# richarddurbin/hash10x

Measured on AMD Instinct MI355X. Metric: read-pairs/s through --readFQB + --hashDepthRange + --cluster (mosh construction + per-barcode clustering), higher is better.
Workload: dtype u64; 1 GPU; yeast-like-2.5M; read_pairs=2500000, barcodes=10000, B=24, k=21, w=31, clusterThreshold=5, parallelism=single GPU

## Files before the change

### hash10x_amd/csrc/stage_c.hip

```cpp
#include "common.hpp"
#include <chrono>
#include "prim.hpp"
#include <type_traits>
#include <rocprim/block/block_radix_sort.hpp>

namespace h10x {


constexpr int CL_THREADS_SMALL = 1024;
constexpr int CL_THREADS_HUGE = 1024;
constexpr u16 NONE16 = 0xFFFF;
constexpr u32 NOHANDLE = 0xFFFFFFFFu;
constexpr int ROWS_IN_FLIGHT = 4;
constexpr int RCHUNK = 4;

__global__ void within_kernel(const u32 *__restrict__ depth, u32 hashNumber, int lo, int hi, u8 *__restrict__ within) {
  const u32 i = blockIdx.x * blockDim.x + threadIdx.x;
  if (i >= hashNumber) return;
  const int n = (int)depth[i];
  if (n >= lo && n < hi) within[i] = 1;
}
__global__ void within_depth_kernel(const u32 *__restrict__ depth, const u8 *__restrict__ within, u32 hashNumber, u32 *__restrict__ out,
                                    const u64 *__restrict__ rowStart, u32 rowShift, u64 *__restrict__ rowInfo ) {
  const u32 i = blockIdx.x * blockDim.x + threadIdx.x;
// ... 182 lines not shown
  const u16 *goodPos; const u32 *nGood;
  const u64 *goodRow;
  const u32 *rows;
  const u32 *list; u32 nList; u32 *workCounter;
  u32 *started;
  const u32 *front; u32 nFront;
  u32 nBlocks; int threshold;
  SegMap segs;
  u32 rowShift;
  u32 nBlocksFirst;
  u32 firstCap;
  u32 hashMinSlots;
  u32 hashBits;
  u16 *handles; size_t handleStride; u32 hStride;
  const u32 *entries;
  u32 *overflow, *overflowCount;
  unsigned char *scratch; size_t scratchStride;
  u32 maxGood;
  u32 ldsBudget;
  u64 *res;
  u64 *stats;
  u64 *phase;
  u32 narrowFirst;
  u32 tpClassT;
};

#define RES_PACK(best, q, tot) ((u64)(best) | ((u64)(q) << 16) | ((u64)(tot) << 40))
constexpr u32 RES_COUNT_MAX = (1u << 24) - 1;
struct Work {
  u16 *first;
  u32 *bm; u16 *pre;
  u16 *root;
  u32 *hist;
  u32 histWords;
};
__host__ __device__ inline size_t pad16(size_t b) { return (b + 15) & ~(size_t)15; }
__host__ __device__ inline size_t workBytes(u32 nFirst, u32 n, u32 nWaves, u32 bmWords) {
  size_t b = pad16((size_t)nFirst * 2) + pad16((size_t)bmWords * 4) + pad16((size_t)bmWords * 2);
  b += pad16((size_t)n * 2);
  b += (size_t)nWaves * (((size_t)n + 3) / 4) * 4;
  return b + 16;
}
constexpr u32 MIN_HIST_WAVES = 5;
constexpr u32 RANKED_FIRST_PER_RANK = 6;
__host__ __device__ inline u32 rankedFirstEstimate(u32 nBarcodes, u32 n) { const u64 e = (u64)RANKED_FIRST_PER_RANK * n; return e < nBarcodes ? (u32)e : nBarcodes; }
__host__ __device__ inline u32 rankedFirstEstimateE(u32 nBarcodes, u32 n, u32 entries, u32 div = 7) { const u32 a = rankedFirstEstimate(nBarcodes, n), b = entries / div; const u32 m = a > b ? a : b; return m < nBarcodes ? m : nBarcodes; }
__host__ __device__ inline u32 histWaves(u32 nFirst, u32 n, u32 maxWaves, u32 bmWords, size_t budget) {
  const size_t fixed = workBytes(nFirst, n, 0, bmWords), per = (((size_t)n + 3) / 4) * 4;
  if (fixed + MIN_HIST_WAVES * per > budget) return 0;
  const size_t wv = (budget - fixed) / (per ? per : 1);
  return wv < maxWaves ? (u32)wv : maxWaves;
}
__device__ inline Work carve(unsigned char *base, u32 nFirst, u32 n, u32 bmWords = 0) {
  Work w; size_t o = 0;
  w.first = (u16 *)(base + o); o += pad16((size_t)nFirst * 2);
  w.bm = (u32 *)(base + o); o += pad16((size_t)bmWords * 4);
  w.pre = (u16 *)(base + o); o += pad16((size_t)bmWords * 2);
  w.root = (u16 *)(base + o); o += pad16((size_t)n * 2);
  w.hist = (u32 *)(base + o); w.histWords = (n + 3) / 4;
  return w;
}
__host__ __device__ inline size_t mergeBytes(u32 nRep) {
  return (((size_t)nRep + 15) & ~(size_t)15) + 256 * 8 * 4 + 256 * 4 + 512 * 4 + 16;
}

template <bool IN_LDS, typename T> __device__ __forceinline__ T ld_shared(const T *p) {
  if (IN_LDS) return *p;
  return __hip_atomic_load(p, __ATOMIC_RELAXED, __HIP_MEMORY_SCOPE_AGENT);
}

template <bool IN_LDS>
__device__ __forceinline__ void min_u16(u16 *arr, u32 idx, u32 val) {
  u32 *w = (u32 *)arr + (idx >> 1); const int sh = (idx & 1) * 16;
  u32 old = ld_shared<IN_LDS>(w);
  for (;;) {
    if (((old >> sh) & 0xFFFFu) <= val) return;
    const u32 nw = (old & ~(0xFFFFu << sh)) | (val << sh);
    const u32 prev = atomicCAS(w, old, nw);
    if (prev == old) return;
    old = prev;
  }
}

template <bool FIRST_LDS> struct FirstDense {
  static constexpr bool MASK_TAIL = false;
  static constexpr bool SELF = true;
  u32 none;
  u16 *first; u32 wide;
  __device__ __forceinline__ u32 update(u32 cj, u32 i) const {
    if (FIRST_LDS && wide) atomicMin(&((u32 *)first)[cj], i); else min_u16<FIRST_LDS>(first, cj, i);
    return cj;
  }
  __device__ __forceinline__ u32 peek(u32 h) const {
    if (FIRST_LDS) return *(const u16 *)((const unsigned char *)first + (u32)(h << (1 + wide)));
    return ld_shared<FIRST_LDS>(&first[h]);
  }
  __device__ __forceinline__ u32 lookup(u32 cj) const { return peek(cj); }
  __device__ __forceinline__ u32 entry(const void *row, u32 j, u32 code) const { const u32 cj = ((const u32 *)row)[j]; return cj != code ? lookup(cj) : (u32)NONE16; }
};
struct FirstRanked {
  static constexpr bool SELF = false;
  static constexpr bool MASK_TAIL = false;
  u16 *first; const u32 *bm; const u16 *pre; u32 wide;
  u32 none;
  __device__ __forceinline__ u32 at(u32 cj) const { const u32 w = cj >> 5; return pre[w] + (u32)__popc(bm[w] & ((1u << (cj & 31)) - 1u)); }
  __device__ __forceinline__ u32 update(u32 cj, u32 i) const { const u32 h = at(cj); if (wide) atomicMin(&((u32 *)first)[h], i); else min_u16<true>(first, h, i); return h; }
  __device__ __forceinline__ u32 peek(u32 h) const { return *(const u16 *)((const unsigned char *)first + (u32)(h << (1 + wide))); }
  __device__ __forceinline__ u32 lookup(u32 cj) const { return peek(at(cj)); }
  __device__ __forceinline__ u32 entry(const void *row, u32 j, u32 code) const { const u32 cj = ((const u32 *)row)[j]; return cj != code ? lookup(cj) : (u32)NONE16; }
};
constexpr u32 TR_QUEUE = 16384;
constexpr u32 TR_MIN_SLOTS = 1024;
constexpr u32 TR_MAX_SLOTS = 65532;
struct SlotTable {
  u32 *tab; u32 NB , xsh , tsh; u32 *ovf; u32 hbase ;
  u32 base3;
  typedef __attribute__((address_space(3))) u32 lds_u32;
  typedef u32 u32x4 __attribute__((ext_vector_type(4)));
  typedef __attribute__((address_space(3))) u32x4 lds_u32x4;
  static constexpr u32 SCRAMBLE = 0x9E3779u;
  static constexpr u32 MAXD = 63;
  static constexpr u32 NOTFOUND = 0xFFFFFFFFu;
  __device__ __forceinline__ void shape(u32 *t, u32 slots, u32 hashBits, u32 *o, u32 hb) {
    tab = t; NB = slots / 4; xsh = 32 - hashBits; ovf = o; hbase = hb; base3 = 0;
    const u32 lg = 31 - (u32)__clz((int)NB), x = 32 - hashBits + lg; tsh = x < 31 ? x : 31;
  }
  __device__ __forceinline__ void inLds() { base3 = (u32)(size_t)(lds_u32 *)tab; }
  __device__ __forceinline__ u32 search(u32 cj, u32 i, bool insert, bool &ins) const {
    const u32 x = __umul24(cj, SCRAMBLE) << xsh;
    u32 b = __umulhi(x, NB);
    const u32 tag = (x * NB) >> tsh;
    const u32 step = 2 * (tag & 7u) + 1;
    ins = false;
    for (u32 key = tag; key < (MAXD << 10); key += 1u << 10) {
      const u32 mine = (i << 16) | key;
      const uint4 e4 = *(const uint4 *)&tab[4 * b];
      const u32 e[4] = {e4.x, e4.y, e4.z, e4.w};
      u32 hit = 4, eh = 0;
#pragma unroll
      for (int w = 3; w >= 0; --w) { const bool m = (e[w] & 0xFFFFu) == key; hit = m ? (u32)w : hit; eh = m ? e[w] : eh; }
      if (hit < 4) { if (eh > (mine | 0xFFFFu)) atomicMin(&tab[4 * b + hit], mine); return hbase + 4 * b + hit; }
#pragma unroll
      for (int w = 0; w < 4; ++w)
        if (e[w] == 0xFFFFFFFFu) {
          if (!insert) return NOTFOUND;
          const u32 old = atomicCAS(&tab[4 * b + w], 0xFFFFFFFFu, mine);
          if (old == 0xFFFFFFFFu) { ins = true; return hbase + 4 * b + w; }
          if ((old & 0xFFFFu) == key) { if (old > (mine | 0xFFFFu)) atomicMin(&tab[4 * b + w], mine); return hbase + 4 * b + w; }
        }
      b += step; if (b >= NB) b -= NB;
    }
    if (insert) *ovf = 1;
    return NOTFOUND;
  }
  __device__ __forceinline__ bool probeHome(u32 cj, u32 i, bool valid , bool insert, u32 &slot, bool &ins) const {
    const u32 x = __umul24(cj, SCRAMBLE) << xsh;
    const u32 b4 = __umulhi(x, NB) << 2;
    const u32 key = (x * NB) >> tsh;
    const u32 mine = (i << 16) | key;
    const u32 aBucket = base3 + (b4 << 2);
    const u32x4 e4 = *(const lds_u32x4 *)(uintptr_t)aBucket;
    const bool m0 = (e4.x & 0xFFFFu) == key, m1 = (e4.y & 0xFFFFu) == key, m2 = (e4.z & 0xFFFFu) == key, m3 = (e4.w & 0xFFFFu) == key;
    const bool z0 = e4.x == 0xFFFFFFFFu, z1 = e4.y == 0xFFFFFFFFu, z2 = e4.z == 0xFFFFFFFFu, z3 = e4.w == 0xFFFFFFFFu;
    const bool hit = m0 | m1 | m2 | m3;
    const u32 wh = m0 ? 0u : (m1 ? 1u : (m2 ? 2u : 3u)), wz = z0 ? 0u : (z1 ? 1u : (z2 ? 2u : 3u));
    const u32 word = hit ? wh : wz;
    slot = b4 | word;
    lds_u32 *const pSlot = (lds_u32 *)(uintptr_t)(aBucket + (word << 2));
    const bool claim = valid && !hit && insert && (z0 | z1 | z2 | z3);
    u32 seen = 0xFFFFFFFEu;
    if (claim) { u32 expect = 0xFFFFFFFFu; __hip_atomic_compare_exchange_strong(pSlot, &expect, mine, __ATOMIC_RELAXED, __ATOMIC_RELAXED, __HIP_MEMORY_SCOPE_WORKGROUP); seen = expect; }
    ins = seen == 0xFFFFFFFFu;
    const bool same = (seen & 0xFFFFu) == key;
    if ((valid && hit) || same) (void)__hip_atomic_fetch_min(pSlot, mine, __ATOMIC_RELAXED, __HIP_MEMORY_SCOPE_WORKGROUP);
    return !valid || hit || ins || same;
  }
};
struct FirstSlots {
  static constexpr bool SELF = false;
  static constexpr bool MASK_TAIL = false;
  const unsigned char *base; u32 sh;
  u32 none;
  __device__ __forceinline__ u32 peek(u32 h) const { return *(const u16 *)(base + (u32)(h << sh)); }
  __device__ __forceinline__ u32 lookup(u32 h) const { return peek(h); }
// ... 89 lines not shown
      }
    }
  if (RCHUNK > 1) {
#pragma unroll
    for (int r = 0; r < RCHUNK; ++r)
      if ((u32)(r * WAVE) < d && ok[r]) {
        if (IN_LDS) hist[f[r] >> 2] = 0;
        else atomicAnd(&hist[f[r] >> 2], 0u);
      }
  }
  if (!(RCHUNK > 2) || __builtin_amdgcn_ballot_w64(key >= (thr << 16))) {
    key = wave_max_u32(key);
    bcnt = key >> 16;
    best = key ? 0xFFFFu - (key & 0xFFFFu) : NONE16;
    if (bcnt >= thr) {
      rb = ld_shared<IN_LDS>(&root[best]);
      if (rb != NONE16) {
#pragma unroll
        for (int r = 0; r < RCHUNK; ++r) if ((u32)(r * WAVE) < d) q += (u32)__popcll(__ballot(f[r] == rb));
      }
    }
  }
}
template <typename FT>
__device__ __forceinline__ u32 row_count_value(const void *__restrict__ row, u32 d, u32 code, u32 i, const FT &ft, u32 v, u32 &tot) {
  const int lane = threadIdx.x & (WAVE - 1);
  u32 q = 0; tot = 0;
  for (u32 b0 = 0; b0 < d; b0 += WAVE) {
    u32 f = NONE16;
    if (b0 + lane < d) f = ft.entry(row, b0 + lane, code);
    q += (u32)__popcll(__ballot(f == v && v != NONE16)); tot += (u32)__popcll(__ballot(f < i));
  }
  return q;
}
template <typename FT>
__device__ __forceinline__ void row_mode_long(const void *__restrict__ row, u32 d, u32 code, u32 i, const FT &ft, u32 &best, u32 &bcnt, u32 &tot) {
  const int lane = threadIdx.x & (WAVE - 1);
  best = NONE16; bcnt = 0; tot = 0;
  for (u32 a0 = 0; a0 < d; a0 += WAVE) {
    u32 fa = NONE16; bool va = false;
    if (a0 + lane < d) { fa = ft.entry(row, a0 + lane, code); va = fa < i; }
    u64 rem = __ballot(va); tot += (u32)__popcll(rem);
    while (rem) {
      const int src = __ffsll((long long)rem) - 1;
      const u32 v = (u32)__builtin_amdgcn_readlane((int)fa, src);
      rem &= ~__ballot(fa == v);
      u32 cnt = 0; bool seenBefore = false;
      for (u32 b0 = 0; b0 < d; b0 += WAVE) {
        u32 fb = NONE16;
        if (b0 + lane < d) fb = ft.entry(row, b0 + lane, code);
        const u32 m = (u32)__popcll(__ballot(fb == v));
        if (b0 < a0 && m) { seenBefore = true; break; }
        cnt += m;
      }
      if (!seenBefore && (cnt > bcnt || (cnt == bcnt && v < best))) { bcnt = cnt; best = v; }
    }
  }
}
#define STAMP(k) do { if (a.phase && threadIdx.x == 0) { const u64 t__ = wall_clock64(); atomicAdd((u64 *)&a.phase[k], t__ - (u64)acc.s[4]); acc.s[4] = t__; } } while (0)

#define SYNC() do { __syncthreads(); if (!IN_LDS) __builtin_amdgcn_fence(__ATOMIC_ACQUIRE, "agent"); } while (0)
#define SYNC_LDS() do { if (IN_LDS) { __builtin_amdgcn_fence(__ATOMIC_RELEASE, "workgroup"); asm volatile("s_waitcnt lgkmcnt(0)\n\ts_barrier" ::: "memory"); __builtin_amdgcn_fence(__ATOMIC_ACQUIRE, "workgroup"); } else SYNC(); } while (0)

struct Desc { u32 x , y ; };
__device__ __forceinline__ Desc descLane(u32 v, int t) { Desc d; d.x = (u32)__builtin_amdgcn_readlane((int)v, t); d.y = (u32)__builtin_amdgcn_readlane((int)v, 32 + t); return d; }
__device__ __forceinline__ u32 descLoad(const u64 *gr, u32 i0, u32 nLists, u32 n) {
  const u32 lane = threadIdx.x & (WAVE - 1), t = lane & 31, i = i0 + t;
  return (t < nLists && i >= 1 && i < n) ? ((const u32 *)gr)[2 * (size_t)i + (lane >> 5)] : 0u;
}

__device__ __forceinline__ u32 descLoadU(const u64 *gr, u32 i0, u32 n) {
  const u32 lane = threadIdx.x & (WAVE - 1), i = i0 + (lane & 31);
  return ((const u32 *)gr)[2 * (size_t)(i < n ? i : n - 1) + (lane >> 5)];
}
__device__ __forceinline__ u32 descFix(u32 v, u32 i0, u32 nLists, u32 n) {
  const u32 lane = threadIdx.x & (WAVE - 1), t = lane & 31, i = i0 + t;
  return (lane < 32 || (t < nLists && i >= 1 && i < n)) ? v : 0u;
}

template <int CL_THREADS> __device__ __forceinline__ void fill16(void *p, size_t bytes, u32 v) {
  const uint4 v4 = make_uint4(v, v, v, v);
  for (u32 i = threadIdx.x; i < (u32)(bytes / 16); i += CL_THREADS) ((uint4 *)p)[i] = v4;
}
struct WorkAcc { u32 depth; unsigned long long *s; };
template <bool IN_LDS, int FIRST_MODE , int CL_THREADS, int KLASS>
__device__ __forceinline__ void cluster_one_block(const ClusterArgs &a, u32 code, unsigned char *region, u16 *firstGlobal, u32 *sh , WorkAcc &acc) {
  constexpr int CL_WAVES = CL_THREADS / WAVE;
  constexpr int RIF = (KLASS == 0 && CL_THREADS == 1024 && FIRST_MODE == 1) ? 2 : ROWS_IN_FLIGHT;
  const int tid = threadIdx.x, lane = tid & (WAVE - 1), wave = tid / WAVE;
  code = (u32)__builtin_amdgcn_readfirstlane((int)code);
  const u32 n = (u32)__builtin_amdgcn_readfirstlane((int)a.nGood[code]);
  if (n == 0) return;
  const u64 o = a.blockOff[code];
  constexpr bool FIRST_LDS = IN_LDS && FIRST_MODE != 2;
  constexpr bool RANKED = IN_LDS && FIRST_MODE == 1;
  const u32 bmWords = RANKED ? (a.nBlocksFirst + 31) / 32 : 0;
  u32 nW;
  if constexpr (RANKED) nW = 0;
  else nW = IN_LDS ? histWaves(FIRST_LDS ? a.nBlocksFirst : 0, n, CL_WAVES, bmWords, a.ldsBudget) : (u32)CL_WAVES;
  if (!RANKED && !nW) return;
  bool wideFirst = false;
  if (FIRST_LDS && !RANKED && a.narrowFirst != 1) {
    const u32 nW4 = histWaves(2 * a.nBlocksFirst, n, CL_WAVES, bmWords, a.ldsBudget);
    wideFirst = nW4 >= nW || (a.narrowFirst >= 2 && nW4 >= a.narrowFirst);
    if (wideFirst) nW = nW4;
  }
  Work w = carve(region, RANKED ? 0 : (FIRST_LDS || !IN_LDS ? (wideFirst ? 2 * a.nBlocksFirst : a.nBlocksFirst) : 0), n, bmWords);
  if (IN_LDS && FIRST_MODE == 2) w.first = firstGlobal;
  typename std::conditional<RANKED, FirstRanked, FirstDense<FIRST_LDS>>::type ft{};
  if constexpr (RANKED) { ft.first = w.first; ft.bm = w.bm; ft.pre = w.pre; ft.wide = 0; }
  else { ft.first = w.first; ft.wide = wideFirst ? 1u : 0u; }
  const u32 lcode = code; code = a.segs.globalOf(lcode);
  if constexpr (!RANKED) ft.none = code;
  const u32 rsh = a.rowShift;
#define ROWP(rs) (a.rows + ((size_t)(rs) << rsh))
  const u64 *const gr = a.goodRow + o;
  u64 *const res = a.res + o;
  const u32 thr = (u32)a.threshold;

  if (a.phase && threadIdx.x == 0) acc.s[4] = wall_clock64();
  if (FIRST_LDS && !RANKED) {
    if (wideFirst) fill16<CL_THREADS>(w.first, pad16((size_t)a.nBlocksFirst * 4), (u32)NONE16);
    else fill16<CL_THREADS>(w.first, pad16((size_t)a.nBlocksFirst * 2), 0xFFFFFFFFu);
  }
  if (RANKED) fill16<CL_THREADS>(w.bm, pad16((size_t)bmWords * 4), 0u);
  if (!RANKED) fill16<CL_THREADS>(w.hist, pad16((size_t)nW * w.histWords * 4), 0u);
  fill16<CL_THREADS>(w.root, pad16((size_t)n * 2), 0xFFFFFFFFu);
  if (tid == 0) { w.root[0] = 0; res[0] = RES_PACK(NONE16, 0, 0); }
  SYNC();
  if constexpr (RANKED) {
    typedef __attribute__((address_space(3))) u32 lds_u32;
    lds_u32 *const bm3 = (lds_u32 *)w.bm;
    auto mark = [&](u32 cj) { if (cj != code) __hip_atomic_fetch_or(&bm3[cj >> 5], 1u << (cj & 31), __ATOMIC_RELAXED, __HIP_MEMORY_SCOPE_WORKGROUP); };
    constexpr int BIF = 8;
    const u32 uw = (u32)__builtin_amdgcn_readfirstlane(wave);
    u32 dvN = descLoad(gr, 1 + uw * BIF, BIF, n);
    for (u32 i0 = 1 + uw * BIF; i0 < n; i0 += CL_WAVES * BIF) {
      u32 c0[BIF], c1[BIF], d4[BIF], r4[BIF];
      const u32 dv = dvN;
      dvN = descLoad(gr, i0 + CL_WAVES * BIF, BIF, n);
#pragma unroll
      for (int t = 0; t < BIF; ++t) {
        const Desc g2 = descLane(dv, t);
        d4[t] = g2.y; r4[t] = g2.x;
        const u32 *row = ROWP(r4[t]);
        c0[t] = (u32)lane < d4[t] ? row[lane] : code; c1[t] = (u32)(WAVE + lane) < d4[t] ? row[WAVE + lane] : code;
      }
#pragma unroll
      for (int t = 0; t < BIF; ++t) {
        mark(c0[t]);
        if (d4[t] > WAVE) {
          mark(c1[t]);
          if (d4[t] > 2 * WAVE) { const u32 *row = ROWP(r4[t]); for (u32 j = 2 * WAVE + lane; j < d4[t]; j += WAVE) mark(row[j]); }
        }
      }
    }
    SYNC();
    const u32 ipt = (bmWords + CL_THREADS - 1) / CL_THREADS, s0 = tid * ipt < bmWords ? tid * ipt : bmWords, s1 = s0 + ipt < bmWords ? s0 + ipt : bmWords;
    u32 mine = 0;
    for (u32 q = s0; q < s1; ++q) mine += (u32)__popc(w.bm[q]);
    u32 inc = mine;
#pragma unroll
    for (int dd = 1; dd < WAVE; dd <<= 1) { const u32 o2 = (u32)__shfl_up((int)inc, dd); if (lane >= dd) inc += o2; }
    if (lane == WAVE - 1) sh[4 + wave] = inc;
    SYNC();
    u32 run = inc - mine, total = 0;
    for (int q = 0; q < CL_WAVES; ++q) { if (q < wave) run += sh[4 + q]; total += sh[4 + q]; }
    for (u32 q = s0; q < s1; ++q) { w.pre[q] = (u16)run; run += (u32)__popc(w.bm[q]); }
    {
      const size_t fixed = workBytes(0, n, 0, bmWords), per = (size_t)w.histWords * 4, need = pad16((size_t)total * 2) + 32;
      const bool fits = total <= 65535u && fixed + need + MIN_HIST_WAVES * per <= a.ldsBudget && !(a.firstCap && total > a.firstCap);
      if (!fits) {
        if (tid == 0) a.overflow[atomicAdd(a.overflowCount, 1u)] = lcode;
        SYNC();
        return;
      }
      const size_t wv = (a.ldsBudget - fixed - need) / (per ? per : 1);
      nW = wv < (size_t)CL_WAVES ? (u32)wv : (u32)CL_WAVES;
      const size_t need4 = pad16((size_t)total * 4) + 32;
      ft.wide = (a.narrowFirst != 1 && fixed + need4 + (size_t)nW * per <= a.ldsBudget) ? 1u : 0u;
      w.first = (u16 *)((unsigned char *)w.hist + pad16((size_t)nW * per));
      ft.first = w.first;
    }
    for (u32 i = tid; i < nW * w.histWords; i += CL_THREADS) w.hist[i] = 0;
    ft.none = total;
    if (ft.wide) for (u32 q = tid; q <= total; q += CL_THREADS) ((u32 *)w.first)[q] = NONE16;
    else for (u32 q = tid; q < (total + 2) / 2; q += CL_THREADS) ((u32 *)w.first)[q] = 0xFFFFFFFFu;
    SYNC();
  }
  STAMP(0);

#define H10X_LOAD_D(I0, DV) { DV = descLoad(gr, (I0), RIF, n); }
#define H10X_LOAD_A(CJ, DV)                                                                                   \
  { _Pragma("unroll") for (int t = 0; t < RIF; ++t) { const Desc g2 = descLane(DV, t); CJ[t] = (u32)lane < g2.y ? ROWP(g2.x)[lane] : code; } }
#define H10X_LOAD_B(CJ2, DV)                                                                                  \
  { _Pragma("unroll") for (int t = 0; t < RIF; ++t) { const Desc g2 = descLane(DV, t); CJ2[t] = (u32)(WAVE + lane) < g2.y ? ROWP(g2.x)[WAVE + lane] : code; } }
  nW = (u32)__builtin_amdgcn_readfirstlane((int)nW);
  const u32 uwave = (u32)__builtin_amdgcn_readfirstlane(wave);
  const bool listWave = uwave < nW;
  const u32 stepR = nW * RIF;
  u32 cjN[RIF], cj2N[RIF], cjNN[RIF];
  u32 dvCur, dvN, dvNN, dvD;
  u32 sDepth = 0;
  H10X_LOAD_D(listWave ? uwave * RIF : n, dvN)
  H10X_LOAD_D(listWave ? uwave * RIF + stepR : n, dvNN)
  H10X_LOAD_D(listWave ? uwave * RIF + 2 * stepR : n, dvD)
  H10X_LOAD_A(cjN, dvN)
  H10X_LOAD_B(cj2N, dvN)
  H10X_LOAD_A(cjNN, dvNN)
  for (u32 r0 = 0; r0 < n; r0 += stepR) {
    const u32 i0 = listWave ? r0 + uwave * RIF : n;
    u32 cj[RIF], cj2[RIF], dl[RIF];
    dvCur = dvN; dvN = dvNN; dvNN = dvD;
#pragma unroll
    for (int t = 0; t < RIF; ++t) { cj[t] = cjN[t]; cj2[t] = cj2N[t]; cjN[t] = cjNN[t]; dl[t] = (u32)__builtin_amdgcn_readlane((int)dvCur, 32 + t); }
    if constexpr (FIRST_MODE != 0) H10X_LOAD_B(cj2N, dvN) else
    if (__builtin_amdgcn_ballot_w64(lane >= 32 && dvN > (u32)WAVE)) H10X_LOAD_B(cj2N, dvN)
    H10X_LOAD_A(cjNN, dvNN)
    H10X_LOAD_D(listWave ? i0 + 3 * stepR : n, dvD)
#define RS_OF(t) ((u32)__builtin_amdgcn_readlane((int)dvCur, t))
#pragma unroll
    for (int t = 0; t < RIF; ++t) {
      const u32 i = i0 + t;
      using FTT = decltype(ft);
      if constexpr (FTT::SELF) { if (cj[t] != code) ft.update(cj[t], i); }
      else cj[t] = cj[t] != code ? ft.update(cj[t], i) : ft.none;
      if (dl[t] > WAVE) {
        if constexpr (FTT::SELF) { if (cj2[t] != code) ft.update(cj2[t], i); }
        else cj2[t] = cj2[t] != code ? ft.update(cj2[t], i) : ft.none;
        if (dl[t] > 2 * WAVE) { const u32 *row = ROWP(RS_OF(t)); for (u32 j = 2 * WAVE + lane; j < dl[t]; j += WAVE) { const u32 c2 = row[j]; if (c2 != code) ft.update(c2, i); } }
      }
    }
    SYNC_LDS();
    constexpr u32 NOENTRY = NOHANDLE;
    u32 rootV = 0; u64 resV = 0; bool mine = false;
#pragma unroll
    for (int t = 0; t < RIF; ++t) {
      const u32 i = i0 + t;
      if (dl[t]) {
        const u32 d = dl[t];
        u32 best, bcnt, tot, rb, q;
        if (d <= WAVE) row_mode_hist<IN_LDS, 1>(nullptr, cj[t], NOENTRY, d, code, i, ft, w.hist + wave * w.histWords, w.root, thr, best, bcnt, tot, rb, q);
        else if (d <= 2 * WAVE) row_mode_hist<IN_LDS, 2>(nullptr, cj[t], cj2[t], d, code, i, ft, w.hist + wave * w.histWords, w.root, thr, best, bcnt, tot, rb, q);
        else if (d < RCHUNK * WAVE) row_mode_hist<IN_LDS, RCHUNK>(ROWP(RS_OF(t)), cj[t], cj2[t], d, code, i, ft, w.hist + wave * w.histWords, w.root, thr, best, bcnt, tot, rb, q);
        else {
          row_mode_long(ROWP(RS_OF(t)), d, code, i, ft, best, bcnt, tot); rb = NONE16; q = 0;
          if (bcnt >= thr) { rb = ld_shared<IN_LDS>(&w.root[best]); if (rb != NONE16) { u32 t2; q = row_count_value(ROWP(RS_OF(t)), d, code, i, ft, rb, t2); } }
        }
        const bool act = bcnt >= thr;
        if (lane == 0) { w.root[i] = act ? (u16)rb : (u16)i; res[i] = RES_PACK(act ? best : NONE16, q, tot); }
        sDepth += d;
      }
    }
    (void)rootV; (void)resV; (void)mine;
  }
#undef RS_OF
#undef H10X_LOAD_D
#undef H10X_LOAD_A
#undef H10X_LOAD_B
  STAMP(1);
  SYNC();
  STAMP(2);

  {
    u16 *todo = (u16 *)w.hist;
    if (tid == 0) sh[2] = 0;
    SYNC();
      for (u32 i0 = 0; i0 < n; i0 += CL_THREADS) {
        const u32 i = i0 + tid;
        bool need = false;
        if (i >= 1 && i < n) need = ld_shared<IN_LDS>(&w.root[i]) == NONE16;
        const u64 bal = __ballot(need);
        if (bal) {
          u32 base = 0;
          if (lane == 0) base = atomicAdd(&sh[2], (u32)__popcll(bal));
          base = (u32)__shfl((int)base, 0);
          if (need) todo[base + (u32)__popcll(bal & ((1ULL << lane) - 1))] = (u16)i;
        }
      }
    SYNC();
    const u32 nTodo = sh[2];
    for (u32 k = tid; k < nTodo; k += CL_THREADS) {
      const u32 i = ld_shared<IN_LDS>(&todo[k]);
      u32 r = (u32)(__hip_atomic_load(&res[i], __ATOMIC_RELAXED, __HIP_MEMORY_SCOPE_AGENT) & 0xFFFFu);
      for (u32 hop = 0; hop < n && r < n; ++hop) {
        const u32 rr = ld_shared<IN_LDS>(&w.root[r]);
        if (rr != NONE16) { r = rr; break; }
        r = (u32)(__hip_atomic_load(&res[r], __ATOMIC_RELAXED, __HIP_MEMORY_SCOPE_AGENT) & 0xFFFFu);
      }
      w.root[i] = (u16)r;
    }
    SYNC();
    STAMP(3);
    const u32 uw = (u32)__builtin_amdgcn_readfirstlane(wave);
    for (u32 k0 = uw * RIF; k0 < nTodo; k0 += CL_WAVES * RIF) {
      u32 ii[RIF], cj[RIF], cjB[RIF], dl[RIF], rsv[RIF], qv[RIF];
#pragma unroll
      for (int t = 0; t < RIF; ++t) {
        const bool on = k0 + t < nTodo;
        ii[t] = (u32)__builtin_amdgcn_readfirstlane((int)(on ? (u32)ld_shared<IN_LDS>(&todo[k0 + t]) : 0u));
        qv[t] = on ? (u32)ld_shared<IN_LDS>(&w.root[ii[t]]) : NONE16;
        const u64 g2 = gr[ii[t]];
        dl[t] = on ? (u32)__builtin_amdgcn_readfirstlane((int)(u32)(g2 >> 32)) : 0u; rsv[t] = (u32)__builtin_amdgcn_readfirstlane((int)(u32)g2);
        const u32 *row = ROWP(rsv[t]);
        cj[t] = (u32)lane < dl[t] ? row[lane] : code; cjB[t] = (u32)(WAVE + lane) < dl[t] ? row[WAVE + lane] : code;
      }
#pragma unroll
      for (int t = 0; t < RIF; ++t) {
        if (dl[t] == 0) continue;
        const u32 i = ii[t];
        u32 f = cj[t] != code ? ft.lookup(cj[t]) : NONE16;
        u32 q = (u32)__popcll(__ballot(f == qv[t])), tt = (u32)__popcll(__ballot(f < i));
        if (dl[t] > WAVE) { f = cjB[t] != code ? ft.lookup(cjB[t]) : NONE16; q += (u32)__popcll(__ballot(f == qv[t])); tt += (u32)__popcll(__ballot(f < i)); }
        if (dl[t] > 2 * WAVE) { const u32 *row = ROWP(rsv[t]); for (u32 b0 = 2 * WAVE; b0 < dl[t]; b0 += WAVE) { f = NONE16; if (b0 + lane < dl[t]) { const u32 c2 = row[b0 + lane]; if (c2 != code) f = ft.lookup(c2); } q += (u32)__popcll(__ballot(f == qv[t])); tt += (u32)__popcll(__ballot(f < i)); } }
        if (lane == 0) res[i] = RES_PACK(__hip_atomic_load(&res[i], __ATOMIC_RELAXED, __HIP_MEMORY_SCOPE_AGENT) & 0xFFFFu, q, tt);
      }
    }
  }
  STAMP(4);

  if (lane == 0) acc.depth += sDepth;
  if (tid == 0) { acc.s[3] += (u32)(gr[0] >> 32); acc.s[0] += n; acc.s[1] += a.blocks[lcode].nHash; acc.s[2] += 1; }
  if (!FIRST_LDS) {
    SYNC();
    const u32 uw = (u32)__builtin_amdgcn_readfirstlane(wave);
    for (u32 i = 1 + uw; i < n; i += CL_WAVES) {
      const u64 g2 = gr[i]; const u32 d = (u32)__builtin_amdgcn_readfirstlane((int)(u32)(g2 >> 32)); const u32 *row = ROWP((u32)__builtin_amdgcn_readfirstlane((int)(u32)g2));
      for (u32 j = lane; j < d; j += WAVE) w.first[row[j]] = NONE16;
    }
  }
  SYNC();
  STAMP(5);
}


template <int CL_THREADS, int KLASS>
__device__ __forceinline__ void cluster_one_block_tr(const ClusterArgs &a, u32 code, unsigned char *region, u32 *sh, WorkAcc &acc) {
  constexpr bool IN_LDS = true;
  constexpr int CL_WAVES = CL_THREADS / WAVE;
  constexpr int RIF = KLASS == 2 ? 8 : ROWS_IN_FLIGHT;
  const int tid = threadIdx.x, lane = tid & (WAVE - 1), wave = tid / WAVE;
  code = (u32)__builtin_amdgcn_readfirstlane((int)code);
  const u32 n = (u32)__builtin_amdgcn_readfirstlane((int)a.nGood[code]);
  if (n == 0) return;
  const u64 o = a.blockOff[code];
  const u32 lcode = code; code = a.segs.globalOf(lcode);
  u32 S, S2, nW; bool compact;
  translatedShape(n, CL_WAVES, a.ldsBudget, a.hashMinSlots, a.entries[lcode], a.nBlocksFirst, a.firstCap, S, S2, nW, compact);
  if (!S || nW < MIN_HIST_WAVES) {
    if (tid == 0) a.overflow[atomicAdd(a.overflowCount, 1u)] = lcode;
    return;
  }
  const u32 closeAt = translatedCloseAt(S, S2);
  auto shFill = [&]() { typedef __attribute__((address_space(3))) u32 lds_u32; return *(volatile lds_u32 *)(lds_u32 *)&sh[1]; };
  const u32 rsh = a.rowShift;
#define ROWP(rs) (a.rows + ((size_t)(rs) << rsh))
  const u64 *const gr = a.goodRow + o;
  u64 *const res = a.res + o;
  u32 thr = (u32)a.threshold;
  asm volatile("" : "+s"(thr));
  u16 *const hs = a.handles + (size_t)blockIdx.x * a.handleStride;
  const u32 hst = a.hStride, lgH = 31 - (u32)__clz((int)hst);
  const u32 uwave = (u32)__builtin_amdgcn_readfirstlane(wave);
  if (a.phase && threadIdx.x == 0) acc.s[4] = wall_clock64();

  u32 *const tab = (u32 *)region;
  for (u32 i = tid; i <= S; i += CL_THREADS) tab[i] = 0xFFFFFFFFu;
  if (tid == 0) { sh[0] = 0; sh[1] = 0; sh[2] = 0; res[0] = RES_PACK(NONE16, 0, 0); }
  SYNC();
  STAMP(0);
  unsigned long long *const queue = (unsigned long long *)(hs + a.handleStride - (size_t)CL_WAVES * TR_QUEUE * 4) + (size_t)uwave * TR_QUEUE;
  u32 qn = 0;
  SlotTable st; st.shape(tab, S, a.hashBits, &sh[2], 0); st.inLds();
  u32 qk = 0;
  auto settle = [&](const SlotTable &t, bool mayInsert, u32 fillLimit, bool all) {
    u32 k0 = qk;
    for (; all ? k0 < qn : k0 + WAVE <= qn; k0 += WAVE) {
      const bool on = k0 + lane < qn;
      const unsigned long long e = on ? queue[k0 + lane] : 0ull;
      const bool insert = mayInsert && shFill() < fillLimit;
      u32 h = 0; bool ins = false;
      if (on) { const u32 dest = (u32)(e >> 22); h = t.search((u32)e & 0x3FFFFFu, dest >> lgH, insert, ins); if (h != SlotTable::NOTFOUND) hs[dest] = (u16)h; }
      const u64 balI = __ballot(ins);
      if (balI && lane == 0) atomicAdd(&sh[1], (u32)__popcll(balI));
      const u64 balU = __ballot(on && h == SlotTable::NOTFOUND);
      if (balU) {
        if (on && h == SlotTable::NOTFOUND) queue[qk + (u32)__popcll(balU & ((1ULL << lane) - 1))] = e;
        qk += (u32)__popcll(balU);
      }
    }
    const u32 rest = k0 < qn ? qn - k0 : 0u;
    if (rest && k0 != qk) { const unsigned long long e = (u32)lane < rest ? queue[k0 + lane] : 0ull; if ((u32)lane < rest) queue[qk + lane] = e; }
    qn = qk + rest;
  };
  {
    bool insert = true;
    u32 myIns = 0;
    const u32 laneU = (u32)lane;
    auto place = [&](u32 cj, u32 i, u32 drem , u16 *hl, u32 dest0) {
      const bool valid = laneU < drem && cj != code;
      u32 slot; bool ins;
      const bool done = st.probeHome(cj, i, valid, insert, slot, ins);
      hl[laneU] = (u16)(valid ? slot : S);
      myIns += (u32)__popcll(__ballot(ins));
// ... 741 lines not shown
        base = (u32)__shfl((int)base, 0);
        if (need) todo[base + (u32)__popcll(bal & ((1ULL << lane) - 1))] = (u16)i;
      }
    }
    SYNC();
    const u32 nTodo = sh[2];
    u64 *const res = a.res + o;
    if (a.phase && tid == 0) { atomicAdd((u64 *)&a.phase[6], (u64)nTodo); atomicAdd((u64 *)&a.phase[7], (u64)n); }
    u16 *const todoBest = todo + nTodo;
    for (u32 k = tid; k < nTodo; k += CL_THREADS) {
      const u32 i = todo[k];
      u32 r = (u32)(__hip_atomic_load(&res[i], __ATOMIC_RELAXED, __HIP_MEMORY_SCOPE_AGENT) & 0xFFFFu);
      todoBest[k] = (u16)r;
      for (u32 hop = 0; hop < n && r < n; ++hop) {
        const u32 rr = *(volatile u16 *)&root[r];
        if (rr != NONE16) { r = rr; break; }
        r = (u32)(__hip_atomic_load(&res[r], __ATOMIC_RELAXED, __HIP_MEMORY_SCOPE_AGENT) & 0xFFFFu);
      }
      root[i] = (u16)r;
    }
    SYNC();
    constexpr int TIF = ROWS_IN_FLIGHT;
    for (u32 k0 = uwave * TIF; k0 < nTodo; k0 += CL_WAVES * TIF) {
      u32 ii[TIF], hA[TIF], hB[TIF], dl[TIF], qv[TIF], bst[TIF]; u64 g[TIF];
#pragma unroll
      for (int t = 0; t < TIF; ++t) {
        const u32 kk = k0 + (u32)t < nTodo ? k0 + (u32)t : nTodo - 1;
        ii[t] = (u32)__builtin_amdgcn_readfirstlane((int)(u32)todo[kk]);
        bst[t] = (u32)todoBest[kk];
        qv[t] = (u32)root[ii[t]];
      }
#pragma unroll
      for (int t = 0; t < TIF; ++t) g[t] = gr[ii[t]];
#pragma unroll
      for (int t = 0; t < TIF; ++t) {
        const u16 *const hrow = hs + tpPos(tp, ii[t], hst), *const hrow64 = hs + tpPos64(tp, ii[t], hst);
        hA[t] = (u32)hrow[laneU]; hB[t] = (u32)hrow64[laneU];
      }
#pragma unroll
      for (int t = 0; t < TIF; ++t) {
        dl[t] = k0 + (u32)t < nTodo ? (u32)__builtin_amdgcn_readfirstlane((int)(u32)(g[t] >> 32)) : 0u;
        hA[t] = laneU < dl[t] ? hA[t] : S; hB[t] = WAVE + laneU < dl[t] ? hB[t] : S;
      }
#pragma unroll
      for (int t = 0; t < TIF; ++t) {
        if (dl[t] == 0) continue;
        const u32 i = ii[t];
        u32 f = ft.peek(hA[t]);
        u32 q = (u32)__popcll(__ballot(f == qv[t])), tt = (u32)__popcll(__ballot(f < i));
        if (dl[t] > WAVE) { f = ft.peek(hB[t]); q += (u32)__popcll(__ballot(f == qv[t])); tt += (u32)__popcll(__ballot(f < i)); }
        if (dl[t] > 2 * WAVE) { const u16 *const hrow = hs + tpPos(tp, i, hst); for (u32 b0 = 2 * WAVE; b0 < dl[t]; b0 += WAVE) { f = b0 + laneU < dl[t] ? ft.peek(hrow[b0 + laneU]) : (u32)NONE16; q += (u32)__popcll(__ballot(f == qv[t])); tt += (u32)__popcll(__ballot(f < i)); } }
        if (lane == 0) res[i] = RES_PACK(bst[t], q, tt);
      }
    }
  }
  if (tid == 0) { acc.s[3] += a.entries[lcode]; acc.s[0] += n; acc.s[1] += a.blocks[lcode].nHash; acc.s[2] += 1; }
  SYNC();
  STAMP(5);
}

#undef SYNC
#undef SYNC_LDS
#undef ROWP

template <bool IN_LDS, int FIRST_MODE, int CL_THREADS, int KLASS = 0 >
__global__ __launch_bounds__(CL_THREADS) __attribute__((amdgpu_waves_per_eu(KLASS == 0 ? (CL_THREADS == 1024 ? 8 : (CL_THREADS == 768 ? 6 : 4)) : 4)))
void cluster_kernel(ClusterArgs a) {
  extern __shared__ __align__(16) unsigned char smem[];
  __shared__ u32 sh[4 + 128];
  unsigned char *region = IN_LDS ? smem : a.scratch + (size_t)blockIdx.x * a.scratchStride;
  u16 *firstGlobal = (IN_LDS && FIRST_MODE == 2) ? (u16 *)(a.scratch + (size_t)blockIdx.x * a.scratchStride) : nullptr;
  __shared__ unsigned long long accS[5];
  WorkAcc acc{0u, accS};
  if (threadIdx.x < 4) accS[threadIdx.x] = 0;
  if (a.started && threadIdx.x == 0) { __hip_atomic_store(&a.started[blockIdx.x], 1u, __ATOMIC_RELAXED, __HIP_MEMORY_SCOPE_SYSTEM); }
  for (;;) {
    __syncthreads();
    if (threadIdx.x == 0) sh[3] = atomicAdd(a.workCounter, 1u);
    __syncthreads();
    const u32 wi = sh[3];
    if (wi >= a.nFront + a.nList) break;
    if constexpr (FIRST_MODE == 5) cluster_one_block_tp<CL_THREADS, KLASS>(a, wi < a.nFront ? a.front[wi] : a.list[wi - a.nFront], region, sh, acc);
    else if constexpr (FIRST_MODE == 4) cluster_one_block_tr<CL_THREADS, KLASS>(a, wi < a.nFront ? a.front[wi] : a.list[wi - a.nFront], region, sh, acc);
    else cluster_one_block<IN_LDS, FIRST_MODE, CL_THREADS, KLASS>(a, wi < a.nFront ? a.front[wi] : a.list[wi - a.nFront], region, firstGlobal, sh, acc);
  }
  u64 depth = acc.depth;
  for (int s = 32; s; s >>= 1) depth += __shfl_down(depth, s);
  if ((threadIdx.x & (WAVE - 1)) == 0 && depth) atomicAdd((u64 *)&a.stats[1], depth);
  if (threadIdx.x == 0 && accS[2]) { atomicAdd((u64 *)&a.stats[0], (u64)accS[0]); atomicAdd((u64 *)&a.stats[1], (u64)accS[3]); atomicAdd((u64 *)&a.stats[2], (u64)accS[1]); atomicAdd((u64 *)&a.stats[3], (u64)accS[2]); }
}

__global__ __launch_bounds__(256)
void good_rows_kernel(const h10x_clushash *__restrict__ ch, const u64 *__restrict__ blockOff, const u32 *__restrict__ nGood, const u16 *__restrict__ goodPos, u32 nBlocks,
                      const u32 *__restrict__ hashDepth, const u64 *__restrict__ rowStart, u32 rowShift, u64 *__restrict__ goodRow) {
  for (u32 c = blockIdx.x; c < nBlocks; c += gridDim.x) {
    const u32 n = nGood[c]; const u64 o = blockOff[c];
    for (u32 i = threadIdx.x; i < n; i += blockDim.x) {
      const u32 x = ch[o + goodPos[o + i]].hash;
      goodRow[o + i] = (u64)(u32)(rowStart[x] >> rowShift) | ((u64)hashDepth[x] << 32);
    }
  }
}

struct ReplayArgs {
  h10x_block *blocks; const u64 *blockOff; h10x_clushash *clusHash; const u16 *goodPos; const u32 *nGood;
  u64 *res;
  u32 codeMin, span, nLo, nHi;
  const u32 *list;
  unsigned char *scratch; size_t scratchStride;
  u32 *raw;
};
#define SYNC() do { __syncthreads(); if (!IN_LDS) __builtin_amdgcn_fence(__ATOMIC_ACQUIRE, "agent"); } while (0)
template <bool IN_LDS, int THREADS>
__global__ __launch_bounds__(THREADS)
void replay_kernel(ReplayArgs a) {
  extern __shared__ __align__(16) unsigned char smem[];
  __shared__ u32 sh[4 + THREADS / WAVE];
  const int tid = threadIdx.x, lane = tid & (WAVE - 1), wave = tid / WAVE;
  unsigned char *region = IN_LDS ? smem : a.scratch + (size_t)blockIdx.x * a.scratchStride;
  for (u32 wi = blockIdx.x; wi < a.span; wi += gridDim.x) {
    const u32 c = a.list ? a.list[wi] : a.codeMin + wi;
    const u32 n = a.nGood[c];
    if (n == 0 || n <= a.nLo || n > a.nHi) continue;
    const u64 o = a.blockOff[c];
    const size_t col = ((size_t)n * 2 + 15) & ~(size_t)15;
    u16 *bst = (u16 *)region, *ptr = (u16 *)(region + col), *ft = (u16 *)(region + 2 * col), *fl = (u16 *)(region + 3 * col);
    SYNC();
    if (tid == 0) sh[2] = 0;
    for (u32 i0 = tid; i0 < n; i0 += 4 * THREADS) {
      u64 rw[4];
#pragma unroll
      for (int k = 0; k < 4; ++k) { const u32 i = i0 + (u32)k * THREADS; rw[k] = a.res[o + (i < n ? i : n - 1)]; }
#pragma unroll
      for (int k = 0; k < 4; ++k) {
        const u32 i = i0 + (u32)k * THREADS;
        if (i < n) { const u16 m = (u16)(rw[k] & 0xFFFFu); bst[i] = m; ptr[i] = m != NONE16 ? m : (u16)i; ft[i] = NONE16; fl[i] = 0; }
      }
    }
    SYNC();
    for (u32 i = tid; i < n; i += THREADS) {
      const u32 b = ld_shared<IN_LDS>(&bst[i]);
      if (b != NONE16 && b < n && ld_shared<IN_LDS>(&bst[b]) == NONE16) min_u16<IN_LDS>(ft, b, i);
    }
    u32 rounds = 1; while ((1u << rounds) < n) ++rounds;
    SYNC();
    for (u32 r = 0; r <= rounds; ++r) {
      int moved = 0;
      for (u32 i = tid; i < n; i += THREADS) {
        const u32 p = ld_shared<IN_LDS>(&ptr[i]);
        if (p < n) { const u32 pp = IN_LDS ? (u32)*(volatile u16 *)&ptr[p] : (u32)ld_shared<false>(&ptr[p]); if (pp != p) { ptr[i] = (u16)pp; moved = 1; } }
      }
      const int any = __syncthreads_or(moved);
      if (!IN_LDS) __builtin_amdgcn_fence(__ATOMIC_ACQUIRE, "agent");
      if (!any) break;
    }
    for (u32 i = tid; i < n; i += THREADS) { const u32 t = ld_shared<IN_LDS>(&ft[i]); if (t != NONE16) fl[t] = 1; }
    SYNC();
    const u32 ipt = (n + THREADS - 1) / THREADS, s0 = tid * ipt < n ? tid * ipt : n, s1 = s0 + ipt < n ? s0 + ipt : n;
    u32 mine = 0;
    for (u32 i = s0; i < s1; ++i) mine += ld_shared<IN_LDS>(&fl[i]);
    u32 inc = mine;
#pragma unroll
    for (int d = 1; d < WAVE; d <<= 1) { const u32 o2 = (u32)__shfl_up((int)inc, d); if (lane >= d) inc += o2; }
    if (lane == WAVE - 1) sh[4 + wave] = inc;
    __syncthreads();
    u32 run = inc - mine;
// ... 581 lines not shown
```

Baseline: 499.6 million read-pairs/s.

## Specialize wide-first dense clustering and add wave-reduced short-row rounds

Turns the runtime choice between 2-byte and 4-byte first-occurrence tables into a template parameter, dispatched once per barcode, so the wide path compiles without the branch. For wide LDS tables, when every row in flight fits in one wave, a new short_round path updates first entries, counts hits with byte-packed LDS histograms, takes the best cluster by a DPP max reduction across lanes, and writes root/res from lanes 32+. This is meant to replace the per-row ballot loops and serial lane work for short rows with one vectorised pass. It adds code size and register pressure, and the 8-bit packed counters could saturate.

```diff
diff --git a/hash10x_amd/csrc/stage_c.hip b/hash10x_amd/csrc/stage_c.hip
--- a/hash10x_amd/csrc/stage_c.hip
+++ b/hash10x_amd/csrc/stage_c.hip
@@ -288,13 +288,16 @@
   }
 }
 
-template <bool FIRST_LDS> struct FirstDense {
+template <bool FIRST_LDS, bool WIDE = false> struct FirstDense {
+  static_assert(FIRST_LDS || !WIDE, "4-byte entries: LDS only");
   static constexpr bool MASK_TAIL = false;
   static constexpr bool SELF = true;
+  static constexpr bool SHORT_ROUNDS = WIDE;
+  static constexpr u32 wide = WIDE ? 1u : 0u;
   u32 none;
-  u16 *first; u32 wide;
+  u16 *first;
   __device__ __forceinline__ u32 update(u32 cj, u32 i) const {
-    if (FIRST_LDS && wide) atomicMin(&((u32 *)first)[cj], i); else min_u16<FIRST_LDS>(first, cj, i);
+    if (WIDE) atomicMin(&((u32 *)first)[cj], i); else min_u16<FIRST_LDS>(first, cj, i);
     return cj;
   }
   __device__ __forceinline__ u32 peek(u32 h) const {
@@ -306,6 +309,7 @@
 };
 struct FirstRanked {
   static constexpr bool SELF = false;
+  static constexpr bool SHORT_ROUNDS = false;
   static constexpr bool MASK_TAIL = false;
   u16 *first; const u32 *bm; const u16 *pre; u32 wide;
   u32 none;
@@ -561,8 +565,65 @@
   const uint4 v4 = make_uint4(v, v, v, v);
   for (u32 i = threadIdx.x; i < (u32)(bytes / 16); i += CL_THREADS) ((uint4 *)p)[i] = v4;
 }
+#if __has_builtin(__builtin_amdgcn_writelane)
+__device__ __forceinline__ int writelane_u32(int s, int l, int v) { return __builtin_amdgcn_writelane(s, l, v); }
+#else
+extern "C" __device__ int writelane_u32(int s, int l, int v) __asm("llvm.amdgcn.writelane.i32");
+#endif
+template <int RIF, typename FT>
+__device__ __forceinline__ void short_round(const FT &ft, const u32 (&h)[RIF] , u32 dv, u32 i0, u32 *hist, u16 *root, u64 *res, u32 thr) {
+  const u32 lane = threadIdx.x & (WAVE - 1);
+  constexpr u32 I0_CAP = (u32)NONE16 & ~(u32)(RIF - 1);
+  const u32 ib = i0 < I0_CAP ? i0 : I0_CAP;
+  u32 f[RIF], c[RIF], key[RIF];
+  u32 totV = 0, keyV = 0, qV = 0;
+#pragma unroll
+  for (int t = 0; t < RIF; ++t) f[t] = ft.peek(h[t]);
+#pragma unroll
+  for (int t = 0; t < RIF; ++t) {
+    const bool ok = f[t] < ib + t;
+    totV = (u32)writelane_u32((int)__popcll(__builtin_amdgcn_ballot_w64(ok)), 32 + t, (int)totV);
+    c[t] = 0xFFFFFFFFu;
+    if (ok) { c[t] = atomicAdd(&hist[f[t] >> 2], 1u << ((f[t] & 3) * 8)); hist[f[t] >> 2] = 0; }
+  }
+#pragma unroll
+  for (int t = 0; t < RIF; ++t) key[t] = ((((c[t] >> ((f[t] & 3) * 8)) + 1) & 0xFFu) << 16) | (0xFFFFu - f[t]);
+#define H10X_DPP_MAX(ctrl, rowmask) { _Pragma("unroll") for (int t = 0; t < RIF; ++t) { const u32 o = (u32)__builtin_amdgcn_update_dpp(0, (int)key[t], ctrl, rowmask, 0xf, false); key[t] = o > key[t] ? o : key[t]; } }
+  H10X_DPP_MAX(0x111, 0xf)
+  H10X_DPP_MAX(0x112, 0xf)
+  H10X_DPP_MAX(0x114, 0xf)
+  H10X_DPP_MAX(0x118, 0xf)
+  H10X_DPP_MAX(0x142, 0xa)
+  H10X_DPP_MAX(0x143, 0xc)
+#undef H10X_DPP_MAX
+#pragma unroll
+  for (int t = 0; t < RIF; ++t) keyV = (u32)writelane_u32(__builtin_amdgcn_readlane((int)key[t], 63), 32 + t, (int)keyV);
+  const bool live = lane >= 32 && dv != 0;
+  const u32 bcnt = keyV >> 16, best = 0xFFFFu - (keyV & 0xFFFFu);
+  const bool act = live && bcnt >= thr;
+  u32 rbV = NONE16;
+  if (act) rbV = root[best];
+#pragma unroll
+  for (int t = 0; t < RIF; ++t) {
+    const u32 rb = (u32)__builtin_amdgcn_readlane((int)rbV, 32 + t);
+    qV = (u32)writelane_u32((int)__popcll(__builtin_amdgcn_ballot_w64(f[t] == rb)), 32 + t, (int)qV);
+  }
+  if (live) {
+    const u32 i = i0 + lane - 32;
+    const u32 q = rbV != NONE16 ? qV : 0u;
+    root[i] = (u16)(act ? rbV : i);
+    const u32 lo = (act ? best : (u32)NONE16) | (q << 16), hi = (q >> 16) | (totV << 8);
+    res[i] = ((u64)hi << 32) | lo;
+  }
+}
 struct WorkAcc { u32 depth; unsigned long long *s; };
-template <bool IN_LDS, int FIRST_MODE , int CL_THREADS, int KLASS>
+template <int CL_THREADS> __device__ __forceinline__ bool dense_first_wide(const ClusterArgs &a, u32 code) {
+  if (a.narrowFirst == 1) return false;
+  const u32 n = (u32)__builtin_amdgcn_readfirstlane((int)a.nGood[__builtin_amdgcn_readfirstlane((int)code)]);
+  const u32 nW = histWaves(a.nBlocksFirst, n, CL_THREADS / WAVE, 0, a.ldsBudget), nW4 = histWaves(2 * a.nBlocksFirst, n, CL_THREADS / WAVE, 0, a.ldsBudget);
+  return nW4 >= nW || (a.narrowFirst >= 2 && nW4 >= a.narrowFirst);
+}
+template <bool IN_LDS, int FIRST_MODE , int CL_THREADS, int KLASS, bool WIDE = false >
 __device__ __forceinline__ void cluster_one_block(const ClusterArgs &a, u32 code, unsigned char *region, u16 *firstGlobal, u32 *sh , WorkAcc &acc) {
   constexpr int CL_WAVES = CL_THREADS / WAVE;
   constexpr int RIF = (KLASS == 0 && CL_THREADS == 1024 && FIRST_MODE == 1) ? 2 : ROWS_IN_FLIGHT;
@@ -576,19 +637,15 @@
   const u32 bmWords = RANKED ? (a.nBlocksFirst + 31) / 32 : 0;
   u32 nW;
   if constexpr (RANKED) nW = 0;
-  else nW = IN_LDS ? histWaves(FIRST_LDS ? a.nBlocksFirst : 0, n, CL_WAVES, bmWords, a.ldsBudget) : (u32)CL_WAVES;
+  else nW = IN_LDS ? histWaves(FIRST_LDS ? (WIDE ? 2 : 1) * a.nBlocksFirst : 0, n, CL_WAVES, bmWords, a.ldsBudget) : (u32)CL_WAVES;
   if (!RANKED && !nW) return;
-  bool wideFirst = false;
-  if (FIRST_LDS && !RANKED && a.narrowFirst != 1) {
-    const u32 nW4 = histWaves(2 * a.nBlocksFirst, n, CL_WAVES, bmWords, a.ldsBudget);
-    wideFirst = nW4 >= nW || (a.narrowFirst >= 2 && nW4 >= a.narrowFirst);
-    if (wideFirst) nW = nW4;
-  }
+  static_assert(!WIDE || (FIRST_LDS && !RANKED), "4-byte entries by template parameter: the dense placement in LDS");
+  constexpr bool wideFirst = WIDE;
   Work w = carve(region, RANKED ? 0 : (FIRST_LDS || !IN_LDS ? (wideFirst ? 2 * a.nBlocksFirst : a.nBlocksFirst) : 0), n, bmWords);
   if (IN_LDS && FIRST_MODE == 2) w.first = firstGlobal;
-  typename std::conditional<RANKED, FirstRanked, FirstDense<FIRST_LDS>>::type ft{};
+  typename std::conditional<RANKED, FirstRanked, FirstDense<FIRST_LDS, WIDE>>::type ft{};
   if constexpr (RANKED) { ft.first = w.first; ft.bm = w.bm; ft.pre = w.pre; ft.wide = 0; }
-  else { ft.first = w.first; ft.wide = wideFirst ? 1u : 0u; }
+  else ft.first = w.first;
   const u32 lcode = code; code = a.segs.globalOf(lcode);
   if constexpr (!RANKED) ft.none = code;
   const u32 rsh = a.rowShift;
@@ -681,6 +738,8 @@
   u32 cjN[RIF], cj2N[RIF], cjNN[RIF];
   u32 dvCur, dvN, dvNN, dvD;
   u32 sDepth = 0;
+  u32 vDepth = 0;
+  using FTT = decltype(ft);
   H10X_LOAD_D(listWave ? uwave * RIF : n, dvN)
   H10X_LOAD_D(listWave ? uwave * RIF + stepR : n, dvNN)
   H10X_LOAD_D(listWave ? uwave * RIF + 2 * stepR : n, dvD)
@@ -692,16 +751,29 @@
     u32 cj[RIF], cj2[RIF], dl[RIF];
     dvCur = dvN; dvN = dvNN; dvNN = dvD;
 #pragma unroll
-    for (int t = 0; t < RIF; ++t) { cj[t] = cjN[t]; cj2[t] = cj2N[t]; cjN[t] = cjNN[t]; dl[t] = (u32)__builtin_amdgcn_readlane((int)dvCur, 32 + t); }
+    for (int t = 0; t < RIF; ++t) { cj[t] = cjN[t]; cj2[t] = cj2N[t]; cjN[t] = cjNN[t]; if constexpr (!FTT::SHORT_ROUNDS) dl[t] = (u32)__builtin_amdgcn_readlane((int)dvCur, 32 + t); }
     if constexpr (FIRST_MODE != 0) H10X_LOAD_B(cj2N, dvN) else
     if (__builtin_amdgcn_ballot_w64(lane >= 32 && dvN > (u32)WAVE)) H10X_LOAD_B(cj2N, dvN)
     H10X_LOAD_A(cjNN, dvNN)
     H10X_LOAD_D(listWave ? i0 + 3 * stepR : n, dvD)
+    if constexpr (FTT::SHORT_ROUNDS) {
+      if (listWave && !__builtin_amdgcn_ballot_w64(lane >= 32 && dvCur > (u32)WAVE)) {
+#pragma unroll
+        for (int t = 0; t < RIF; ++t) if (cj[t] != code) ft.update(cj[t], i0 + t);
+        SYNC_LDS();
+        short_round<RIF>(ft, cj, dvCur, i0, w.hist + wave * w.histWords, w.root, res, thr);
+        vDepth += lane >= 32 ? dvCur : 0u;
+        continue;
+      }
+    }
 #define RS_OF(t) ((u32)__builtin_amdgcn_readlane((int)dvCur, t))
+    if constexpr (FTT::SHORT_ROUNDS) {
+#pragma unroll
+      for (int t = 0; t < RIF; ++t) dl[t] = (u32)__builtin_amdgcn_readlane((int)dvCur, 32 + t);
+    }
 #pragma unroll
     for (int t = 0; t < RIF; ++t) {
       const u32 i = i0 + t;
-      using FTT = decltype(ft);
       if constexpr (FTT::SELF) { if (cj[t] != code) ft.update(cj[t], i); }
       else cj[t] = cj[t] != code ? ft.update(cj[t], i) : ft.none;
       if (dl[t] > WAVE) {
@@ -712,7 +784,6 @@
     }
     SYNC_LDS();
     constexpr u32 NOENTRY = NOHANDLE;
-    u32 rootV = 0; u64 resV = 0; bool mine = false;
 #pragma unroll
     for (int t = 0; t < RIF; ++t) {
       const u32 i = i0 + t;
@@ -731,7 +802,6 @@
         sDepth += d;
       }
     }
-    (void)rootV; (void)resV; (void)mine;
   }
 #undef RS_OF
 #undef H10X_LOAD_D
@@ -799,6 +869,7 @@
   STAMP(4);
 
   if (lane == 0) acc.depth += sDepth;
+  if constexpr (FTT::SHORT_ROUNDS) acc.depth += vDepth;
   if (tid == 0) { acc.s[3] += (u32)(gr[0] >> 32); acc.s[0] += n; acc.s[1] += a.blocks[lcode].nHash; acc.s[2] += 1; }
   if (!FIRST_LDS) {
     SYNC();
@@ -1706,6 +1777,11 @@
     if (wi >= a.nFront + a.nList) break;
     if constexpr (FIRST_MODE == 5) cluster_one_block_tp<CL_THREADS, KLASS>(a, wi < a.nFront ? a.front[wi] : a.list[wi - a.nFront], region, sh, acc);
     else if constexpr (FIRST_MODE == 4) cluster_one_block_tr<CL_THREADS, KLASS>(a, wi < a.nFront ? a.front[wi] : a.list[wi - a.nFront], region, sh, acc);
+    else if constexpr (IN_LDS && FIRST_MODE == 0) {
+      const u32 code = wi < a.nFront ? a.front[wi] : a.list[wi - a.nFront];
+      if (dense_first_wide<CL_THREADS>(a, code)) cluster_one_block<IN_LDS, FIRST_MODE, CL_THREADS, KLASS, true>(a, code, region, firstGlobal, sh, acc);
+      else cluster_one_block<IN_LDS, FIRST_MODE, CL_THREADS, KLASS, false>(a, code, region, firstGlobal, sh, acc);
+    }
     else cluster_one_block<IN_LDS, FIRST_MODE, CL_THREADS, KLASS>(a, wi < a.nFront ? a.front[wi] : a.list[wi - a.nFront], region, firstGlobal, sh, acc);
   }
   u64 depth = acc.depth;
```

After: 514.7 million read-pairs/s, median of 6. 3.0% higher.
